# GonzaBerger/bmSparse-SPGEMM-SPMV

Hardware: AMD Instinct MI355X
Metric: bmSparse SpMV fp32 effective GB/s (CSR-convention bytes / time); SpGEMM GFLOP/s under `spgemm` (higher is better)
Workload: dtype f32; 1 GPU; bmSparse SpMV fp32, rmat(scale=20, edge_factor=2)+I, stand-in for webbase-1M; rows=1048576, nnz=3127380, blocks=2073692, x=ones, variant=default (value-stream sweep over the cached plan), hbm_resident_copies_rotated=9

## Files before the change

### bmsparse-spgemm-spmv_amd/csrc/spmv.hip

```cpp
#include "spmv_plan.h"
#include "prims.hip.h"
#include <cstdlib>
#include <cstdio>
#include <algorithm>
#include <vector>
#include <type_traits>

namespace bmsp {
namespace {

constexpr uint32_t kVsGroup = 96;
bool vstream_eligible(const bmsp_matrix_s *A)
{
    return !(A->spmv_full_tiles * 4 >= A->block_num) && !getenv("BMSP_SPMV_OLD") && A->num_block_cols() < (1ll << 28);
}

struct RowClass {
    const uint32_t *rowptr;
    const uint64_t *offsets;
    uint32_t nbr;
    uint32_t group;
    __device__ bool is_long(uint32_t r) const { return rowptr[r + 1] - rowptr[r] > kItemTiles; }
    __device__ bool starts(uint32_t r) const
    {
// ... 794 lines not shown
    constexpr int GROUPS = LANES_PER_ROW / 8;
    const uint32_t gid = blockIdx.x * (kThreads / LANES_PER_ROW) + threadIdx.x / LANES_PER_ROW;
    if (gid >= num_block_rows) return;
    const int sub = threadIdx.x % LANES_PER_ROW;
    const int g = sub >> 3, r = sub & 7;
    const uint32_t b0 = rowptr[gid], b1 = rowptr[gid + 1];
    A acc = 0;
    for (uint32_t b = b0 + g; b < b1; b += GROUPS) {
        uint64_t bmp = bmps[b];
        uint32_t byte = tile_byte(bmp, r);
        if (byte) {
            uint32_t before = r ? (uint32_t)__popcll(bmp >> (64 - 8 * r)) : 0u;
            acc = tile_row_dot<T, A>(byte, values + offsets[b] + before, x, key_col(keys[b]) * 8u, num_cols, acc);
        }
    }
    if (GROUPS > 1) {
#pragma unroll
        for (int d = 8; d < LANES_PER_ROW; d <<= 1) acc += __shfl_xor(acc, d, kWave);
    }
    uint32_t row = gid * 8u + (uint32_t)r;
    if (g == 0 && row >= row_lo && row < num_rows) y[row] = acc;
}

template <typename T, int U>
__global__ __launch_bounds__(kThreads) void spmv_rowgroup_kernel(const uint32_t *__restrict__ rowptr, const uint64_t *__restrict__ keys,
                                                                 const uint64_t *__restrict__ bmps, const uint64_t *__restrict__ offsets,
                                                                 const T *__restrict__ values, const T *__restrict__ x,
                                                                 typename Acc<T>::type *__restrict__ y, uint32_t num_rows, uint32_t num_cols,
                                                                 uint32_t nbr, uint32_t values_bytes, uint32_t passes, uint32_t row_lo)
{
    using A = typename Acc<T>::type;
    const int lane = lane_id(), j = lane & 15, g = lane >> 4;
    const uint32_t wv = blockIdx.x * 4 + wave_id();
    const rsrc_t rv = make_rsrc(values, values_bytes), rx = make_rsrc(x, num_cols * (uint32_t)sizeof(T));
    const uint32_t xlane = (uint32_t)((j & 1) * 4);
    const uint32_t bshift = (uint32_t)(60 - 4 * j) & 31u;
    const bool in_hi = j < 8;
    const uint32_t hi_mask = j >= 8 ? 0xffffffffu : (j == 0 ? 0u : 0xffffffffu << (32 - 4 * j));
    const uint32_t lo_mask = j > 8 ? 0xffffffffu << (64 - 4 * j) : 0u;
    const bool ragged_x = (num_cols & 3u) != 0u;
    for (uint32_t p = 0; p < passes; p++) {
        const uint32_t br = (wv * passes + p) * 4u + (uint32_t)g;
        if ((wv * passes + p) * 4u >= nbr) break;
        const bool valid = br < nbr;
        uint32_t t = valid ? rowptr[br] : 0u;
        const uint32_t t1 = valid ? rowptr[br + 1] : 0u;
        A acc = 0;
        uint32_t blo[U], bhi[U], col[U], off[U];
#pragma unroll
        for (int u = 0; u < U; u++) {
            const bool on = t + u < t1;
            const uint64_t bm = on ? bmps[t + u] : 0ull;
            blo[u] = (uint32_t)bm; bhi[u] = (uint32_t)(bm >> 32);
            col[u] = on ? (uint32_t)keys[t + u] : 0u;
            off[u] = on ? (uint32_t)offsets[t + u] : 0u;
        }
        while (__any(t < t1)) {
            A av[U][4], xv[U][4];
            uint32_t nib[U];
#pragma unroll
            for (int u = 0; u < U; u++) {
                nib[u] = ((in_hi ? bhi[u] : blo[u]) >> bshift) & 0xfu;
                const uint32_t rank = (uint32_t)__builtin_popcount(bhi[u] & hi_mask) + (uint32_t)__builtin_popcount(blo[u] & lo_mask);
                const uint32_t vaddr = (off[u] + rank) * (uint32_t)sizeof(T);
                if (sizeof(T) == 2) {
                    typedef uint32_t u32x3 __attribute__((ext_vector_type(3)));
                    typedef _Float16 h2 __attribute__((ext_vector_type(2)));
                    const u32x3 d = __builtin_amdgcn_raw_buffer_load_b96(rv, nib[u] ? (vaddr & ~3u) : kOob, 0, 0);
                    const uint32_t sh = (vaddr & 2u) * 8u;
                    const h2 p0 = __builtin_bit_cast(h2, __builtin_amdgcn_alignbit(d[1], d[0], sh)), p1 = __builtin_bit_cast(h2, __builtin_amdgcn_alignbit(d[2], d[1], sh));
                    av[u][0] = (A)p0[0]; av[u][1] = (A)p0[1]; av[u][2] = (A)p1[0]; av[u][3] = (A)p1[1];
                } else {
                    Buf4<T>::ld(rv, nib[u] ? vaddr : kOob, av[u]);
                }
                const uint32_t xc = col[u] * 8u + xlane;
                if (ragged_x && xc + 4u > num_cols) {
#pragma unroll
                    for (int q = 0; q < 4; q++) xv[u][q] = (A)Buf<T>::ld(rx, nib[u] && xc + q < num_cols ? (xc + q) * (uint32_t)sizeof(T) : kOob);
                } else {
                    Buf4<T>::ld(rx, nib[u] ? xc * (uint32_t)sizeof(T) : kOob, xv[u]);
                }
            }
            uint32_t nlo[U], nhi[U], ncol[U], noff[U];
#pragma unroll
            for (int u = 0; u < U; u++) {
                const bool on = t + U + u < t1;
                const uint64_t bm = on ? bmps[t + U + u] : 0ull;
                nlo[u] = (uint32_t)bm; nhi[u] = (uint32_t)(bm >> 32);
                ncol[u] = on ? (uint32_t)keys[t + U + u] : 0u;
                noff[u] = on ? (uint32_t)offsets[t + U + u] : 0u;
            }
#pragma unroll
            for (int u = 0; u < U; u++) {
                const uint32_t n = nib[u];
                A e0, e1, e2, e3;
                if (__all(n == 0xfu || n == 0u)) {
                    e0 = av[u][0]; e1 = av[u][1]; e2 = av[u][2]; e3 = av[u][3];
                    if (n == 0u) { e0 = e1 = e2 = e3 = A(0); }
                } else {
                    const bool b0 = n & 8u, b1 = n & 4u, b2 = n & 2u, b3 = n & 1u;
                    const uint32_t i2 = (uint32_t)b0 + (uint32_t)b1, i3 = i2 + (uint32_t)b2;
                    e0 = b0 ? av[u][0] : A(0);
                    e1 = b1 ? (b0 ? av[u][1] : av[u][0]) : A(0);
                    e2 = b2 ? (i2 == 0 ? av[u][0] : (i2 == 1 ? av[u][1] : av[u][2])) : A(0);
                    e3 = b3 ? (i3 == 0 ? av[u][0] : (i3 == 1 ? av[u][1] : (i3 == 2 ? av[u][2] : av[u][3]))) : A(0);
                }
                acc += e0 * xv[u][0] + e1 * xv[u][1] + e2 * xv[u][2] + e3 * xv[u][3];
            }
            t += U;
#pragma unroll
            for (int u = 0; u < U; u++) { blo[u] = nlo[u]; bhi[u] = nhi[u]; col[u] = ncol[u]; off[u] = noff[u]; }
        }
        if (sizeof(A) == 4) acc += __builtin_bit_cast(float, __builtin_amdgcn_update_dpp(0, __builtin_bit_cast(int, (float)acc), 0xB1, 0xf, 0xf, false));
        else acc += __shfl_xor(acc, 1, kWave);
        const uint32_t row = br * 8u + (uint32_t)(j >> 1);
        if (valid && !(j & 1) && row >= row_lo && row < num_rows) y[row] = acc;
    }
}

#ifndef BMSP_CH_V
#define BMSP_CH_V 512
#endif
constexpr uint32_t kChV = BMSP_CH_V;
constexpr int kChPer = (int)kChV / 64;
static_assert(kChPer % 4 == 0, "a lane loads its values four at a time");
constexpr uint32_t kChWin = 1024;
constexpr int64_t kChMinChunks = 128;
enum { kChHead = 1, kChTail = 2 };

struct ChunkRec {
    uint32_t fb;
    uint32_t own_b, own_e;
    uint32_t flags;
    uint32_t head_ca, head_cb;
    uint32_t tail_cb;
    uint32_t nwin;
};

__device__ __forceinline__ float chunk_sum8(const float (&s)[8], int lane)
{
    const bool h5 = lane & 32, h4 = lane & 16, h3 = lane & 8;
    float t[4], u[2];
#pragma unroll
    for (int i = 0; i < 4; i++) t[i] = (h5 ? s[i + 4] : s[i]) + __shfl_xor(h5 ? s[i] : s[i + 4], 32, kWave);
#pragma unroll
    for (int i = 0; i < 2; i++) u[i] = (h4 ? t[i + 2] : t[i]) + __shfl_xor(h4 ? t[i] : t[i + 2], 16, kWave);
    float v = (h3 ? u[1] : u[0]) + __shfl_xor(h3 ? u[0] : u[1], 8, kWave);
    v += __shfl_xor(v, 4, kWave);
    v += __shfl_xor(v, 2, kWave);
    v += __shfl_xor(v, 1, kWave);
    return v;
}

__device__ __forceinline__ void chunk_fold(const float *__restrict__ carry, float *__restrict__ y, uint32_t *__restrict__ counters, uint32_t ca,
                                           uint32_t cb, uint32_t br, uint32_t num_rows, int lane)
{
    const int r = lane & 7, g = lane >> 3;
    float sum = 0.f;
    for (uint32_t k = ca + (uint32_t)g; k <= cb; k += 8)
        sum += __hip_atomic_load(&carry[((size_t)k * 2 + (k == ca ? 1 : 0)) * 8 + r], __ATOMIC_RELAXED, __HIP_MEMORY_SCOPE_AGENT);
#pragma unroll
    for (int d = 8; d < 64; d <<= 1) sum += __shfl_xor(sum, d, kWave);
    const uint32_t row = br * 8u + (uint32_t)r;
    if (g == 0 && row < num_rows) y[row] = sum;
    if (lane == 0) __hip_atomic_store(&counters[ca], 0u, __ATOMIC_RELAXED, __HIP_MEMORY_SCOPE_AGENT);
}

__global__ __launch_bounds__(64, 8) void spmv_chunk_kernel(const ChunkRec *__restrict__ recs, const uint32_t *__restrict__ words,
                                                            const float *__restrict__ values, const float *__restrict__ x, float *__restrict__ y,
                                                            float *__restrict__ carry, uint32_t *__restrict__ counters, uint32_t nnz,
                                                            uint32_t num_rows, uint32_t num_cols, uint32_t colbits)
{
    typedef float f4 __attribute__((ext_vector_type(4)));
    typedef uint32_t u4 __attribute__((ext_vector_type(4)));
    __shared__ float win[kChWin];
    const int lane = lane_id();
    const uint32_t c = blockIdx.x;
    const ChunkRec rc = recs[c];
    const uint32_t first = c * kChV + (uint32_t)(kChPer * lane);
    const rsrc_t rw = make_rsrc(words, nnz * 4u), rv = make_rsrc(values, nnz * 4u), rx = make_rsrc(x, num_cols * 4u);
    uint32_t w[kChPer];
    float a[kChPer], xv[kChPer];
    if (c * kChV + kChV <= nnz) {
#pragma unroll
        for (int q = 0; q < kChPer; q += 4) {
            const u4 wq = __builtin_bit_cast(u4, __builtin_amdgcn_raw_buffer_load_b128(rw, (first + q) * 4u, 0, 0));
            const f4 aq = __builtin_bit_cast(f4, __builtin_amdgcn_raw_buffer_load_b128(rv, (first + q) * 4u, 0, 0));
#pragma unroll
            for (int i = 0; i < 4; i++) { w[q + i] = wq[i]; a[q + i] = aq[i]; }
        }
    } else {
#pragma unroll
        for (int j = 0; j < kChPer; j++) {
            const uint32_t off = first + j < nnz ? (first + j) * 4u : kOob;
            w[j] = __builtin_amdgcn_raw_buffer_load_b32(rw, off, 0, 0);
            a[j] = Buf<float>::ld(rv, off);
        }
    }
    const uint32_t cmask = (1u << colbits) - 1u;
#pragma unroll
    for (int j = 0; j < kChPer; j++) xv[j] = Buf<float>::ld(rx, first + j < nnz ? (w[j] & cmask) * 4u : kOob);

    float pr[kChPer];
    uint32_t rr[kChPer];
#pragma unroll
    for (int j = 0; j < kChPer; j++) {
        rr[j] = w[j] >> colbits;
        pr[j] = first + j < nnz ? a[j] * xv[j] : 0.f;
    }
    if (rc.nwin == 8) {
        float s[8] = {0.f, 0.f, 0.f, 0.f, 0.f, 0.f, 0.f, 0.f};
#pragma unroll
        for (int j = 0; j < kChPer; j++) {
#pragma unroll
            for (int k = 0; k < 8; k++) s[k] += rr[j] == (uint32_t)k ? pr[j] : 0.f;
        }
        const float v = chunk_sum8(s, lane);
        if ((lane & 7) == 0) win[((lane >> 5) & 1) * 4 + ((lane >> 4) & 1) * 2 + ((lane >> 3) & 1)] = v;
    } else {
        for (uint32_t e = (uint32_t)lane; e < rc.nwin; e += 64) win[e] = 0.f;
        __builtin_amdgcn_wave_barrier();
        float acc[kChPer];
        bool lead[kChPer];
#pragma unroll
        for (int j = 0; j < kChPer; j++) acc[j] = pr[j];
#pragma unroll
        for (int j = 0; j < kChPer; j++) {
            bool taken = false;
#pragma unroll
            for (int i = 0; i < j; i++) {
                const bool hit = !taken && rr[i] == rr[j];
                acc[i] += hit ? acc[j] : 0.f;
                taken |= hit;
            }
            lead[j] = !taken;
        }
#pragma unroll
        for (int j = 0; j < kChPer; j++)
            if (lead[j] && first + j < nnz) lds_add(win + rr[j], acc[j]);
    }
    __builtin_amdgcn_wave_barrier();
    const int32_t base = (int32_t)(rc.fb * 8u);
    const uint32_t row_end = min(rc.own_e * 8u, num_rows);
    for (uint32_t row = rc.own_b * 8u + (uint32_t)lane; row < row_end; row += 64) {
        const int32_t rel = (int32_t)row - base;
        y[row] = rel >= 0 && rel < (int32_t)rc.nwin ? win[rel] : 0.f;
    }
    if (!rc.flags) return;
    if ((rc.flags & kChHead) && lane < 8) __hip_atomic_store(&carry[((size_t)c * 2) * 8 + lane], win[lane], __ATOMIC_RELAXED, __HIP_MEMORY_SCOPE_AGENT);
    if ((rc.flags & kChTail) && lane < 8)
        __hip_atomic_store(&carry[((size_t)c * 2 + 1) * 8 + lane], win[rc.nwin - 8u + (uint32_t)lane], __ATOMIC_RELAXED, __HIP_MEMORY_SCOPE_AGENT);
    asm volatile("s_waitcnt vmcnt(0)" ::: "memory");
    uint32_t ticket = 0;
    if (lane == 0 && (rc.flags & kChHead)) ticket = __hip_atomic_fetch_add(&counters[rc.head_ca], 1u, __ATOMIC_RELAXED, __HIP_MEMORY_SCOPE_AGENT);
    if (lane == 1 && (rc.flags & kChTail)) ticket = __hip_atomic_fetch_add(&counters[c], 1u, __ATOMIC_RELAXED, __HIP_MEMORY_SCOPE_AGENT);
    const uint32_t th = (uint32_t)__builtin_amdgcn_readlane((int)ticket, 0), tt = (uint32_t)__builtin_amdgcn_readlane((int)ticket, 1);
    if ((rc.flags & kChHead) && th == rc.head_cb - rc.head_ca) chunk_fold(carry, y, counters, rc.head_ca, rc.head_cb, rc.fb, num_rows, lane);
    if ((rc.flags & kChTail) && tt == rc.tail_cb - c) chunk_fold(carry, y, counters, c, rc.tail_cb, rc.fb + rc.nwin / 8u - 1u, num_rows, lane);
}

__global__ void chunk_bounds_kernel(const uint64_t *__restrict__ keys, const uint64_t *__restrict__ bmps, const uint64_t *__restrict__ offsets,
                                    uint32_t nb, uint32_t nnz, uint32_t *__restrict__ fbr, uint32_t *__restrict__ lbr)
{
    const uint32_t b = blockIdx.x * blockDim.x + threadIdx.x;
    if (b >= nb) return;
    const uint32_t o = (uint32_t)offsets[b], n = (uint32_t)__popcll(bmps[b]);
    if (n == 0) return;
    const uint32_t br = key_row(keys[b]);
    for (uint32_t c = (o + kChV - 1) / kChV; c * kChV < o + n; c++) fbr[c] = br;
    for (uint32_t c = o / kChV; c <= (o + n - 1) / kChV; c++) {
        const uint32_t e = min((c + 1) * kChV, nnz) - 1u;
        if (e >= o && e < o + n) lbr[c] = br;
    }
}

__global__ void chunk_words_kernel(const uint64_t *__restrict__ keys, const uint64_t *__restrict__ bmps, const uint64_t *__restrict__ offsets,
                                   uint32_t nb, const uint32_t *__restrict__ fbr, uint32_t colbits, uint32_t *__restrict__ words)
{
    const uint32_t b = blockIdx.x * blockDim.x + threadIdx.x;
    if (b >= nb) return;
    uint64_t bm = bmps[b];
    const uint64_t k = keys[b];
    const uint32_t br = key_row(k), bc = key_col(k);
    uint32_t idx = (uint32_t)offsets[b];
    while (bm) {
        const uint32_t p = (uint32_t)__clzll((long long)bm);
        bm &= ~(0x8000000000000000ull >> p);
        const uint32_t rel = (br - fbr[idx / kChV]) * 8u + (p >> 3);
        words[idx] = (rel << colbits) | (bc * 8u + (p & 7u));
        idx++;
    }
}

void build_chunk_cache(bmsp_matrix_s *A, hipStream_t st)
{
    if (A->spmv_cw || A->spmv_cw_tried) return;
    A->spmv_cw_tried = 1;
    if (A->dtype != BMSP_F32 || A->view_values_end || A->view_block_begin || A->nnz == 0 || A->nnz >= (1ll << 30) || A->block_num == 0) return;
    if ((uintptr_t)A->values & 15u) return;
    const uint32_t nnz = (uint32_t)A->nnz, nb = (uint32_t)A->block_num;
    const uint32_t nch = (nnz + kChV - 1) / kChV;
    const int colbits = A->num_cols <= 1 ? 1 : 32 - __builtin_clz((uint32_t)A->num_cols - 1u);
    if (colbits > 28) return;
    std::vector<uint32_t> fb(nch), lb(nch);
    {
        DevBuf<uint32_t> d(2 * (size_t)nch);
        hipLaunchKernelGGL(chunk_bounds_kernel, dim3((nb + 255) / 256), dim3(256), 0, st, A->keys, A->bmps, A->offsets, nb, nnz, d.p, d.p + nch);
        BMSP_CHECK_LAUNCH();
        BMSP_HIP(hipStreamSynchronize(st));
        copy_d2h_staged(fb.data(), d.p, 4 * (size_t)nch);
        copy_d2h_staged(lb.data(), d.p + nch, 4 * (size_t)nch);
    }
    const uint64_t row_cap = std::min<uint64_t>(kChWin, 1ull << (32 - colbits));
    std::vector<ChunkRec> rec(nch);
    const uint32_t nbr = (uint32_t)A->num_block_rows();
    int64_t split = 0;
    for (uint32_t c = 0; c < nch; c++) {
        ChunkRec &r = rec[c];
        r.fb = fb[c];
        r.nwin = (lb[c] - fb[c] + 1u) * 8u;
        if (lb[c] < fb[c] || r.nwin > row_cap) return;
        const bool head = c > 0 && lb[c - 1] == fb[c], tail = c + 1 < nch && fb[c + 1] == lb[c];
        r.own_b = c == 0 ? 0u : fb[c] + (head ? 1u : 0u);
        r.own_e = c + 1 < nch ? fb[c + 1] : nbr;
        r.flags = (head ? kChHead : 0) | (tail && !(head && fb[c] == lb[c]) ? kChTail : 0);
        r.head_ca = r.head_cb = r.tail_cb = c;
    }
    for (uint32_t c = 0; c < nch; c++) {
        if (!(rec[c].flags & kChTail)) continue;
        split++;
        uint32_t e = c + 1;
        while (e + 1 < nch && fb[e + 1] == lb[c]) e++;
        rec[c].tail_cb = e;
        for (uint32_t k = c + 1; k <= e; k++) { rec[k].head_ca = c; rec[k].head_cb = e; }
    }
    const size_t off_rec = (size_t)nch * kChV * 4, off_cnt = off_rec + sizeof(ChunkRec) * (size_t)nch;
    const size_t off_carry = (off_cnt + 4 * (size_t)nch + 63) & ~size_t(63), total = off_carry + 64 * (size_t)nch;
    char *mem = (char *)pool_alloc(total);
    BMSP_HIP(hipMemsetAsync(mem, 0, total, st));
    BMSP_HIP(hipMemcpyAsync(mem + off_rec, rec.data(), sizeof(ChunkRec) * (size_t)nch, hipMemcpyHostToDevice, st));
    {
        DevBuf<uint32_t> d(nch);
        BMSP_HIP(hipMemcpyAsync(d.p, fb.data(), 4 * (size_t)nch, hipMemcpyHostToDevice, st));
        hipLaunchKernelGGL(chunk_words_kernel, dim3((nb + 255) / 256), dim3(256), 0, st, A->keys, A->bmps, A->offsets, nb, d.p, (uint32_t)colbits, (uint32_t *)mem);
        BMSP_CHECK_LAUNCH();
        BMSP_HIP(hipStreamSynchronize(st));
    }
    A->spmv_cw = (uint32_t *)mem;
    A->spmv_cw_chunks = nch;
    A->spmv_cw_split = split;
    A->spmv_cw_off_rec = off_rec; A->spmv_cw_off_cnt = off_cnt; A->spmv_cw_off_carry = off_carry;
    A->spmv_cw_colbits = colbits;
}

bool chunk_wanted(const bmsp_matrix_s *A, uint32_t row_lo, uint32_t row_hi)
{
    if (A->dtype != BMSP_F32 || row_lo != 0 || row_hi != (uint32_t)A->num_rows || A->view_values_end || A->view_block_begin) return false;
    if (getenv("BMSP_SPMV_NOCHUNK") || getenv("BMSP_SPMV_NO_POSCACHE") || getenv("BMSP_SPMV_RED")) return false;
    if (getenv("BMSP_SPMV_CHUNK")) return true;
    return A->nnz < 2 * A->block_num && (A->nnz + kChV - 1) / kChV >= kChMinChunks;
}

template <typename T>
void launch(bmsp_matrix_s *A, const void *v, void *u, int variant, hipStream_t st, uint32_t row_lo, uint32_t row_hi)
{
    using Ac = typename Acc<T>::type;
    uint32_t nbr = (uint32_t)A->num_block_rows();
    if (nbr == 0) return;
    if (variant == BMSP_SPMV_BATCHED) {
        hipLaunchKernelGGL((spmv_blockrow_kernel<T, 64>), dim3((nbr + 3) / 4), dim3(kThreads), 0, st, A->rowptr, A->keys, A->bmps,
                           A->offsets, (const T *)A->values, (const T *)v, (Ac *)u, row_hi,
                           (uint32_t)A->num_cols, nbr, row_lo);
    } else if (variant == 2) {
        hipLaunchKernelGGL((spmv_blockrow_kernel<T, 8>), dim3((nbr + 31) / 32), dim3(kThreads), 0, st, A->rowptr, A->keys, A->bmps,
                           A->offsets, (const T *)A->values, (const T *)v, (Ac *)u, row_hi,
                           (uint32_t)A->num_cols, nbr, row_lo);
    } else if ((size_t)A->values_extent() * sizeof(T) >= (1ull << 32) || (size_t)A->num_cols * sizeof(T) >= (1ull << 32)) {
        hipLaunchKernelGGL((spmv_blockrow_kernel<T, 64>), dim3((nbr + 3) / 4), dim3(kThreads), 0, st, A->rowptr, A->keys, A->bmps,
                           A->offsets, (const T *)A->values, (const T *)v, (Ac *)u, row_hi,
                           (uint32_t)A->num_cols, nbr, row_lo);
    } else {
        build_plan(A, st);
        const bool dense_tiles = A->block_num > 0 && A->nnz >= 16 * A->block_num;
        if ((variant == 3 || (variant == BMSP_SPMV_DEFAULT && dense_tiles && A->spmv_plan_long == 0 && !getenv("BMSP_SPMV_NO_ROWGROUP"))) && pool_owns(A->values)) {
            constexpr int U = 3;
            const uint32_t groups = (nbr + 3) / 4;
            const char *pe = getenv("BMSP_SPMV_PASSES");
            const uint32_t passes = pe ? (uint32_t)std::max(1, atoi(pe)) : (groups > 32768 ? 2u : 1u);
            const uint32_t waves = (groups + passes - 1) / passes;
            hipLaunchKernelGGL((spmv_rowgroup_kernel<T, U>), dim3((waves + 3) / 4), dim3(kThreads), 0, st, A->rowptr, A->keys, A->bmps, A->offsets,
                               (const T *)A->values, (const T *)v, (Ac *)u, row_hi, (uint32_t)A->num_cols, nbr,
                               (uint32_t)((size_t)A->values_extent() * sizeof(T)) + 16u, passes, row_lo);
// ... 145 lines not shown
```

Baseline: 2645 GB/s.

## Replace per-lane LDS atomic adds with DPP segmented reduction in chunk SpMV

In the multi-row chunk path, the per-lane O(kChPer^2) duplicate-combining loop followed by LDS atomic adds is replaced with a block-row (8-row) segmented reduction. Each lane builds 8-wide partial vectors per block row, runs a DPP-based segmented scan across the wave keyed on the last block row, and writes complete block rows to LDS with 16-byte vector stores instead of atomics. Out-of-range tail elements get a dummy row key so they do not break segments. This is meant to cut LDS atomic traffic and serialization, at the cost of more VALU and DPP work and an assumption that each lane's elements are sorted by row. A standalone experiment harness is also added that compares the two variants.

Result: faster. 2843 GB/s, median of 6 (+7.5%).

```diff
diff --git a/bmsparse-spgemm-spmv_amd/csrc/spmv.hip b/bmsparse-spgemm-spmv_amd/csrc/spmv.hip
--- a/bmsparse-spgemm-spmv_amd/csrc/spmv.hip
+++ b/bmsparse-spgemm-spmv_amd/csrc/spmv.hip
@@ -970,6 +970,65 @@
     return v;
 }
 
+__device__ __forceinline__ void chunk_put8(float *p, const float (&v)[8])
+{
+    typedef float f4 __attribute__((ext_vector_type(4)));
+    *(f4 *)p = f4{v[0], v[1], v[2], v[3]};
+    *(f4 *)(p + 4) = f4{v[4], v[5], v[6], v[7]};
+}
+
+template <int CTRL, int ROWS>
+__device__ __forceinline__ bool chunk_scan_step(float (&t)[8], uint32_t key)
+{
+    const bool m = dpp_u32<CTRL, ROWS>(~0u, key) == key;
+    if (!__builtin_amdgcn_ballot_w64(m)) return false;
+#pragma unroll
+    for (int k = 0; k < 8; k++) {
+        const float n = t[k] + dpp_val<CTRL, ROWS>(0.f, t[k]);
+        t[k] = m ? n : t[k];
+    }
+    return true;
+}
+
+__device__ __forceinline__ void chunk_seg_reduce(float *win, const uint32_t (&rk)[kChPer], const float (&pr)[kChPer])
+{
+    const uint32_t bf = rk[0] >> 3, bl = rk[kChPer - 1] >> 3;
+    float h[8], t[8];
+#pragma unroll
+    for (int k = 0; k < 8; k++) h[k] = t[k] = 0.f;
+#pragma unroll
+    for (int j = 0; j < kChPer; j++) {
+        if (j > 0 && (rk[j] >> 3) != (rk[j - 1] >> 3)) {
+            const uint32_t bp = rk[j - 1] >> 3;
+            if (bp == bf) {
+#pragma unroll
+                for (int k = 0; k < 8; k++) h[k] = t[k];
+            } else {
+                chunk_put8(win + 8u * bp, t);
+            }
+#pragma unroll
+            for (int k = 0; k < 8; k++) t[k] = 0.f;
+        }
+        const uint32_t r = rk[j] & 7u;
+#pragma unroll
+        for (int k = 0; k < 8; k++) t[k] += r == (uint32_t)k ? pr[j] : 0.f;
+    }
+    if (chunk_scan_step<0x111, 0xf>(t, bl) && chunk_scan_step<0x112, 0xf>(t, bl) && chunk_scan_step<0x114, 0xf>(t, bl)) chunk_scan_step<0x118, 0xf>(t, bl);
+    chunk_scan_step<0x142, 0xa>(t, bl);
+    chunk_scan_step<0x143, 0xc>(t, bl);
+    const uint32_t bl_left = dpp_u32<0x138>(~0u, bl), bf_right = dpp_u32<0x130>(~0u, bf);
+    float tl[8];
+#pragma unroll
+    for (int k = 0; k < 8; k++) tl[k] = dpp_val<0x138>(0.f, t[k]);
+    if (bf != bl) {
+        const bool cont = bl_left == bf;
+#pragma unroll
+        for (int k = 0; k < 8; k++) h[k] = cont ? h[k] + tl[k] : h[k];
+        chunk_put8(win + 8u * bf, h);
+    }
+    if (bf_right != bl) chunk_put8(win + 8u * bl, t);
+}
+
 __device__ __forceinline__ void chunk_fold(const float *__restrict__ carry, float *__restrict__ y, uint32_t *__restrict__ counters, uint32_t ca,
                                            uint32_t cb, uint32_t br, uint32_t num_rows, int lane)
 {
@@ -991,7 +1050,7 @@
 {
     typedef float f4 __attribute__((ext_vector_type(4)));
     typedef uint32_t u4 __attribute__((ext_vector_type(4)));
-    __shared__ float win[kChWin];
+    __shared__ __attribute__((aligned(16))) float win[kChWin];
     const int lane = lane_id();
     const uint32_t c = blockIdx.x;
     const ChunkRec rc = recs[c];
@@ -1023,7 +1082,7 @@
     uint32_t rr[kChPer];
 #pragma unroll
     for (int j = 0; j < kChPer; j++) {
-        rr[j] = w[j] >> colbits;
+        rr[j] = first + j < nnz ? w[j] >> colbits : rc.nwin - 8u;
         pr[j] = first + j < nnz ? a[j] * xv[j] : 0.f;
     }
     if (rc.nwin == 8) {
@@ -1038,24 +1097,7 @@
     } else {
         for (uint32_t e = (uint32_t)lane; e < rc.nwin; e += 64) win[e] = 0.f;
         __builtin_amdgcn_wave_barrier();
-        float acc[kChPer];
-        bool lead[kChPer];
-#pragma unroll
-        for (int j = 0; j < kChPer; j++) acc[j] = pr[j];
-#pragma unroll
-        for (int j = 0; j < kChPer; j++) {
-            bool taken = false;
-#pragma unroll
-            for (int i = 0; i < j; i++) {
-                const bool hit = !taken && rr[i] == rr[j];
-                acc[i] += hit ? acc[j] : 0.f;
-                taken |= hit;
-            }
-            lead[j] = !taken;
-        }
-#pragma unroll
-        for (int j = 0; j < kChPer; j++)
-            if (lead[j] && first + j < nnz) lds_add(win + rr[j], acc[j]);
+        chunk_seg_reduce(win, rr, pr);
     }
     __builtin_amdgcn_wave_barrier();
     const int32_t base = (int32_t)(rc.fb * 8u);
diff --git a/experiments/spmv_chunk_segscan.hip b/experiments/spmv_chunk_segscan.hip
--- /dev/null
+++ b/experiments/spmv_chunk_segscan.hip
@@ -0,0 +1,405 @@
+#include <hip/hip_runtime.h>
+#include <algorithm>
+#include <cmath>
+#include <cstdint>
+#include <cstdio>
+#include <vector>
+
+constexpr uint32_t kV = 512, kPer = kV / 64, kWin = 1024, kOob = 0xffffffffu;
+enum { kHead = 1, kTail = 2 };
+struct Rec { uint32_t fb, own_b, own_e, flags, head_ca, head_cb, tail_cb, nwin; };
+typedef __amdgpu_buffer_rsrc_t rsrc_t;
+typedef float f4 __attribute__((ext_vector_type(4)));
+typedef uint32_t u4 __attribute__((ext_vector_type(4)));
+
+__device__ __forceinline__ rsrc_t rsrc(const void *p, uint32_t bytes) { return __builtin_amdgcn_make_buffer_rsrc(const_cast<void *>(p), 0, bytes, 0x00020000); }
+__device__ __forceinline__ float ldf(rsrc_t r, uint32_t off) { return __builtin_bit_cast(float, __builtin_amdgcn_raw_buffer_load_b32(r, off, 0, 0)); }
+
+__device__ __forceinline__ float sum8(const float (&s)[8], int lane)
+{
+    const bool h5 = lane & 32, h4 = lane & 16, h3 = lane & 8;
+    float t[4], u[2];
+#pragma unroll
+    for (int i = 0; i < 4; i++) t[i] = (h5 ? s[i + 4] : s[i]) + __shfl_xor(h5 ? s[i] : s[i + 4], 32, 64);
+#pragma unroll
+    for (int i = 0; i < 2; i++) u[i] = (h4 ? t[i + 2] : t[i]) + __shfl_xor(h4 ? t[i] : t[i + 2], 16, 64);
+    float v = (h3 ? u[1] : u[0]) + __shfl_xor(h3 ? u[0] : u[1], 8, 64);
+    v += __shfl_xor(v, 4, 64);
+    v += __shfl_xor(v, 2, 64);
+    v += __shfl_xor(v, 1, 64);
+    return v;
+}
+
+__device__ __forceinline__ void fold(const float *carry, float *y, uint32_t *counters, uint32_t ca, uint32_t cb, uint32_t br, uint32_t num_rows, int lane)
+{
+    const int r = lane & 7, g = lane >> 3;
+    float sum = 0.f;
+    for (uint32_t k = ca + (uint32_t)g; k <= cb; k += 8)
+        sum += __hip_atomic_load(&carry[((size_t)k * 2 + (k == ca ? 1 : 0)) * 8 + r], __ATOMIC_RELAXED, __HIP_MEMORY_SCOPE_AGENT);
+#pragma unroll
+    for (int d = 8; d < 64; d <<= 1) sum += __shfl_xor(sum, d, 64);
+    const uint32_t row = br * 8u + (uint32_t)r;
+    if (g == 0 && row < num_rows) y[row] = sum;
+    if (lane == 0) __hip_atomic_store(&counters[ca], 0u, __ATOMIC_RELAXED, __HIP_MEMORY_SCOPE_AGENT);
+}
+
+__device__ __forceinline__ void load_chunk(uint32_t c, int lane, const uint32_t *words, const float *values, const float *x, uint32_t nnz,
+                                           uint32_t num_cols, uint32_t (&w)[kPer], float (&a)[kPer], float (&xv)[kPer])
+{
+    const uint32_t first = c * kV + kPer * (uint32_t)lane;
+    const rsrc_t rw = rsrc(words, nnz * 4u), rv = rsrc(values, nnz * 4u), rx = rsrc(x, num_cols * 4u);
+    if (c * kV + kV <= nnz) {
+#pragma unroll
+        for (uint32_t q = 0; q < kPer; q += 4) {
+            const u4 wq = __builtin_bit_cast(u4, __builtin_amdgcn_raw_buffer_load_b128(rw, (first + q) * 4u, 0, 0));
+            const f4 aq = __builtin_bit_cast(f4, __builtin_amdgcn_raw_buffer_load_b128(rv, (first + q) * 4u, 0, 0));
+#pragma unroll
+            for (int i = 0; i < 4; i++) { w[q + i] = wq[i]; a[q + i] = aq[i]; }
+        }
+    } else {
+#pragma unroll
+        for (uint32_t j = 0; j < kPer; j++) {
+            const uint32_t off = first + j < nnz ? (first + j) * 4u : kOob;
+            w[j] = __builtin_amdgcn_raw_buffer_load_b32(rw, off, 0, 0);
+            a[j] = ldf(rv, off);
+        }
+    }
+#pragma unroll
+    for (uint32_t j = 0; j < kPer; j++) xv[j] = ldf(rx, first + j < nnz ? (w[j] & 0xfffffu) * 4u : kOob);
+}
+
+template <int R, bool CMB = false>
+__global__ __launch_bounds__(64, 8) void r5_kernel(const Rec *recs, const uint32_t *words, const float *values, const float *x, float *y, float *out,
+                                                   float *carry, uint32_t *counters, uint32_t nnz, uint32_t num_rows, uint32_t num_cols)
+{
+    __shared__ float win[kWin];
+    const int lane = threadIdx.x & 63;
+    const uint32_t c = blockIdx.x;
+    const Rec rc = recs[c];
+    const uint32_t first = c * kV + kPer * (uint32_t)lane;
+    uint32_t w[kPer];
+    float a[kPer], xv[kPer];
+    load_chunk(c, lane, words, values, x, nnz, num_cols, w, a, xv);
+    if (rc.nwin == 8) {
+        float s[8] = {0.f, 0.f, 0.f, 0.f, 0.f, 0.f, 0.f, 0.f};
+#pragma unroll
+        for (uint32_t j = 0; j < kPer; j++) {
+            const uint32_t rr = w[j] >> 20;
+            const float p = first + j < nnz ? a[j] * xv[j] : 0.f;
+#pragma unroll
+            for (int k = 0; k < 8; k++) s[k] += rr == (uint32_t)k ? p : 0.f;
+        }
+        const float v = sum8(s, lane);
+        if ((lane & 7) == 0) win[((lane >> 5) & 1) * 4 + ((lane >> 4) & 1) * 2 + ((lane >> 3) & 1)] = v;
+    } else {
+        for (uint32_t e = (uint32_t)lane; e < rc.nwin; e += 64) win[e] = 0.f;
+        __builtin_amdgcn_wave_barrier();
+        if constexpr (CMB) {
+            float acc[kPer];
+            bool lead[kPer];
+#pragma unroll
+            for (uint32_t j = 0; j < kPer; j++) acc[j] = first + j < nnz ? a[j] * xv[j] : 0.f;
+#pragma unroll
+            for (uint32_t j = 0; j < kPer; j++) {
+                bool taken = false;
+#pragma unroll
+                for (uint32_t i = 0; i < j; i++) {
+                    const bool hit = !taken && (w[i] >> 20) == (w[j] >> 20);
+                    acc[i] += hit ? acc[j] : 0.f;
+                    taken |= hit;
+                }
+                lead[j] = !taken;
+            }
+#pragma unroll
+            for (uint32_t j = 0; j < kPer; j++)
+                if (lead[j] && first + j < nnz) __hip_atomic_fetch_add(win + (w[j] >> 20), acc[j], __ATOMIC_RELAXED, __HIP_MEMORY_SCOPE_WAVEFRONT);
+        }
+        float run = 0.f;
+#pragma unroll
+        for (uint32_t j = 0; j < kPer && !CMB; j++) {
+            const uint32_t rr = w[j] >> 20;
+            const bool on = first + j < nnz;
+            const bool flush = j == kPer - 1 || first + j + 1 >= nnz || (w[j + (j < kPer - 1 ? 1 : 0)] >> 20) != rr;
+            run += on ? a[j] * xv[j] : 0.f;
+            if (flush) {
+                if (on) __hip_atomic_fetch_add(win + rr, run, __ATOMIC_RELAXED, __HIP_MEMORY_SCOPE_WAVEFRONT);
+                run = 0.f;
+            }
+        }
+    }
+    __builtin_amdgcn_wave_barrier();
+    if constexpr (R == 2) {
+        out[c * 64 + lane] = win[lane & 7];
+        return;
+    }
+    const int32_t base = (int32_t)(rc.fb * 8u);
+    const uint32_t row_end = min(rc.own_e * 8u, num_rows);
+    for (uint32_t row = rc.own_b * 8u + (uint32_t)lane; row < row_end; row += 64) {
+        const int32_t rel = (int32_t)row - base;
+        y[row] = rel >= 0 && rel < (int32_t)rc.nwin ? win[rel] : 0.f;
+    }
+    if (R == 3 || !rc.flags) return;
+    if ((rc.flags & kHead) && lane < 8) __hip_atomic_store(&carry[((size_t)c * 2) * 8 + lane], win[lane], __ATOMIC_RELAXED, __HIP_MEMORY_SCOPE_AGENT);
+    if ((rc.flags & kTail) && lane < 8)
+        __hip_atomic_store(&carry[((size_t)c * 2 + 1) * 8 + lane], win[rc.nwin - 8u + (uint32_t)lane], __ATOMIC_RELAXED, __HIP_MEMORY_SCOPE_AGENT);
+    asm volatile("s_waitcnt vmcnt(0)" ::: "memory");
+    if constexpr (R == 4) return;
+    uint32_t ticket = 0;
+    if (lane == 0 && (rc.flags & kHead)) ticket = __hip_atomic_fetch_add(&counters[rc.head_ca], 1u, __ATOMIC_RELAXED, __HIP_MEMORY_SCOPE_AGENT);
+    if (lane == 1 && (rc.flags & kTail)) ticket = __hip_atomic_fetch_add(&counters[c], 1u, __ATOMIC_RELAXED, __HIP_MEMORY_SCOPE_AGENT);
+    const uint32_t th = (uint32_t)__builtin_amdgcn_readlane((int)ticket, 0), tt = (uint32_t)__builtin_amdgcn_readlane((int)ticket, 1);
+    if constexpr (R == 5) {
+        if (th == kOob && tt == kOob) out[c * 64 + lane] = 0.f;
+        return;
+    }
+    if ((rc.flags & kHead) && th == rc.head_cb - rc.head_ca) fold(carry, y, counters, rc.head_ca, rc.head_cb, rc.fb, num_rows, lane);
+    if ((rc.flags & kTail) && tt == rc.tail_cb - c) fold(carry, y, counters, c, rc.tail_cb, rc.fb + rc.nwin / 8u - 1u, num_rows, lane);
+}
+
+template <int CTRL, int ROWS = 0xf>
+__device__ __forceinline__ float dppf(float old, float v)
+{
+    return __builtin_bit_cast(float, __builtin_amdgcn_update_dpp(__builtin_bit_cast(int, old), __builtin_bit_cast(int, v), CTRL, ROWS, 0xf, false));
+}
+template <int CTRL, int ROWS = 0xf>
+__device__ __forceinline__ uint32_t dppu(uint32_t old, uint32_t v) { return (uint32_t)__builtin_amdgcn_update_dpp((int)old, (int)v, CTRL, ROWS, 0xf, false); }
+
+__device__ __forceinline__ void put8(float *p, const float (&v)[8])
+{
+    *(f4 *)p = f4{v[0], v[1], v[2], v[3]};
+    *(f4 *)(p + 4) = f4{v[4], v[5], v[6], v[7]};
+}
+
+template <int CTRL, int ROWS>
+__device__ __forceinline__ bool seg_step(float (&t)[8], uint32_t key)
+{
+    const bool m = dppu<CTRL, ROWS>(~0u, key) == key;
+    if (!__builtin_amdgcn_ballot_w64(m)) return false;
+#pragma unroll
+    for (int k = 0; k < 8; k++) {
+        const float n = t[k] + dppf<CTRL, ROWS>(0.f, t[k]);
+        t[k] = m ? n : t[k];
+    }
+    return true;
+}
+
+__device__ __forceinline__ void seg_reduce(float *win, const uint32_t (&rk)[kPer], const float (&pr)[kPer])
+{
+    const uint32_t bf = rk[0] >> 3, bl = rk[kPer - 1] >> 3;
+    float h[8], t[8];
+#pragma unroll
+    for (int k = 0; k < 8; k++) h[k] = t[k] = 0.f;
+#pragma unroll
+    for (uint32_t j = 0; j < kPer; j++) {
+        if (j > 0 && (rk[j] >> 3) != (rk[j - 1] >> 3)) {
+            const uint32_t bp = rk[j - 1] >> 3;
+            if (bp == bf) {
+#pragma unroll
+                for (int k = 0; k < 8; k++) h[k] = t[k];
+            } else {
+                put8(win + 8u * bp, t);
+            }
+#pragma unroll
+            for (int k = 0; k < 8; k++) t[k] = 0.f;
+        }
+        const uint32_t r = rk[j] & 7u;
+#pragma unroll
+        for (int k = 0; k < 8; k++) t[k] += r == (uint32_t)k ? pr[j] : 0.f;
+    }
+    if (seg_step<0x111, 0xf>(t, bl) && seg_step<0x112, 0xf>(t, bl) && seg_step<0x114, 0xf>(t, bl)) seg_step<0x118, 0xf>(t, bl);
+    seg_step<0x142, 0xa>(t, bl);
+    seg_step<0x143, 0xc>(t, bl);
+    const uint32_t bl_left = dppu<0x138>(~0u, bl), bf_right = dppu<0x130>(~0u, bf);
+    float tl[8];
+#pragma unroll
+    for (int k = 0; k < 8; k++) tl[k] = dppf<0x138>(0.f, t[k]);
+    if (bf != bl) {
+        const bool cont = bl_left == bf;
+#pragma unroll
+        for (int k = 0; k < 8; k++) h[k] = cont ? h[k] + tl[k] : h[k];
+        put8(win + 8u * bf, h);
+    }
+    if (bf_right != bl) put8(win + 8u * bl, t);
+}
+
+__global__ __launch_bounds__(64, 8) void r7_kernel(const Rec *recs, const uint32_t *words, const float *values, const float *x, float *y,
+                                                   float *carry, uint32_t *counters, uint32_t nnz, uint32_t num_rows, uint32_t num_cols)
+{
+    __shared__ __attribute__((aligned(16))) float win[kWin];
+    const int lane = threadIdx.x & 63;
+    const uint32_t c = blockIdx.x;
+    const Rec rc = recs[c];
+    const uint32_t first = c * kV + kPer * (uint32_t)lane;
+    uint32_t w[kPer];
+    float a[kPer], xv[kPer];
+    load_chunk(c, lane, words, values, x, nnz, num_cols, w, a, xv);
+    float pr[kPer];
+    uint32_t rr[kPer];
+#pragma unroll
+    for (uint32_t j = 0; j < kPer; j++) {
+        rr[j] = first + j < nnz ? w[j] >> 20 : rc.nwin - 8u;
+        pr[j] = first + j < nnz ? a[j] * xv[j] : 0.f;
+    }
+    if (rc.nwin == 8) {
+        float s[8] = {0.f, 0.f, 0.f, 0.f, 0.f, 0.f, 0.f, 0.f};
+#pragma unroll
+        for (uint32_t j = 0; j < kPer; j++)
+#pragma unroll
+            for (int k = 0; k < 8; k++) s[k] += rr[j] == (uint32_t)k ? pr[j] : 0.f;
+        const float v = sum8(s, lane);
+        if ((lane & 7) == 0) win[((lane >> 5) & 1) * 4 + ((lane >> 4) & 1) * 2 + ((lane >> 3) & 1)] = v;
+    } else {
+        for (uint32_t e = (uint32_t)lane; e < rc.nwin; e += 64) win[e] = 0.f;
+        __builtin_amdgcn_wave_barrier();
+        seg_reduce(win, rr, pr);
+    }
+    __builtin_amdgcn_wave_barrier();
+    const int32_t base = (int32_t)(rc.fb * 8u);
+    const uint32_t row_end = min(rc.own_e * 8u, num_rows);
+    for (uint32_t row = rc.own_b * 8u + (uint32_t)lane; row < row_end; row += 64) {
+        const int32_t rel = (int32_t)row - base;
+        y[row] = rel >= 0 && rel < (int32_t)rc.nwin ? win[rel] : 0.f;
+    }
+    if (!rc.flags) return;
+    if ((rc.flags & kHead) && lane < 8) __hip_atomic_store(&carry[((size_t)c * 2) * 8 + lane], win[lane], __ATOMIC_RELAXED, __HIP_MEMORY_SCOPE_AGENT);
+    if ((rc.flags & kTail) && lane < 8)
+        __hip_atomic_store(&carry[((size_t)c * 2 + 1) * 8 + lane], win[rc.nwin - 8u + (uint32_t)lane], __ATOMIC_RELAXED, __HIP_MEMORY_SCOPE_AGENT);
+    asm volatile("s_waitcnt vmcnt(0)" ::: "memory");
+    uint32_t ticket = 0;
+    if (lane == 0 && (rc.flags & kHead)) ticket = __hip_atomic_fetch_add(&counters[rc.head_ca], 1u, __ATOMIC_RELAXED, __HIP_MEMORY_SCOPE_AGENT);
+    if (lane == 1 && (rc.flags & kTail)) ticket = __hip_atomic_fetch_add(&counters[c], 1u, __ATOMIC_RELAXED, __HIP_MEMORY_SCOPE_AGENT);
+    const uint32_t th = (uint32_t)__builtin_amdgcn_readlane((int)ticket, 0), tt = (uint32_t)__builtin_amdgcn_readlane((int)ticket, 1);
+    if ((rc.flags & kHead) && th == rc.head_cb - rc.head_ca) fold(carry, y, counters, rc.head_ca, rc.head_cb, rc.fb, num_rows, lane);
+    if ((rc.flags & kTail) && tt == rc.tail_cb - c) fold(carry, y, counters, c, rc.tail_cb, rc.fb + rc.nwin / 8u - 1u, num_rows, lane);
+}
+
+#define CK(x)                                                                                 \
+    do {                                                                                      \
+        hipError_t e_ = (x);                                                                  \
+        if (e_ != hipSuccess) { printf("HIP error %s at line %d\n", hipGetErrorString(e_), __LINE__); return 1; } \
+    } while (0)
+
+int main()
+{
+    const uint32_t scale = 20, n = 1u << scale, m = 2u << scale, copies = 9;
+    uint64_t z = 12345;
+    auto next = [&z]() { z = z * 6364136223846793005ull + 1442695040888963407ull; return (double)(z >> 11) * (1.0 / 9007199254740992.0); };
+    std::vector<uint64_t> cells;
+    for (uint32_t e = 0; e < m + n; e++) {
+        uint32_t r = 0, c = 0;
+        if (e < m) {
+            for (uint32_t l = 0; l < scale; l++) {
+                const double u = next();
+                r = (r << 1) | (u >= 0.76 ? 1u : 0u);
+                c = (c << 1) | (((u >= 0.57 && u < 0.76) || u >= 0.95) ? 1u : 0u);
+            }
+        } else {
+            r = c = e - m;
+        }
+        cells.push_back(((uint64_t)(r >> 3) << 43) | ((uint64_t)(c >> 3) << 26) | ((uint64_t)(((r & 7u) << 3) | (c & 7u)) << 20) | c);
+    }
+    std::sort(cells.begin(), cells.end());
+    cells.erase(std::unique(cells.begin(), cells.end()), cells.end());
+    const uint32_t nnz = (uint32_t)cells.size(), nch = (nnz + kV - 1) / kV, nbr = n / 8;
+    auto brow = [&](uint32_t i) { return (uint32_t)(cells[i] >> 43); };
+    std::vector<uint32_t> fb(nch), lb(nch);
+    for (uint32_t c = 0; c < nch; c++) { fb[c] = brow(c * kV); lb[c] = brow(std::min((c + 1) * kV, nnz) - 1); }
+    std::vector<Rec> rec(nch);
+    uint32_t hub = 0, folded = 0;
+    for (uint32_t c = 0; c < nch; c++) {
+        Rec &r = rec[c];
+        r.fb = fb[c];
+        r.nwin = (lb[c] - fb[c] + 1u) * 8u;
+        if (r.nwin > kWin) { printf("chunk %u spans %u rows: beyond the window\n", c, r.nwin); return 1; }
+        const bool head = c > 0 && lb[c - 1] == fb[c], tail = c + 1 < nch && fb[c + 1] == lb[c];
+        r.own_b = c == 0 ? 0u : fb[c] + (head ? 1u : 0u);
+        r.own_e = c + 1 < nch ? fb[c + 1] : nbr;
+        r.flags = (head ? kHead : 0) | (tail && !(head && fb[c] == lb[c]) ? kTail : 0);
+        r.head_ca = r.head_cb = r.tail_cb = c;
+        hub += r.nwin == 8;
+        folded += r.flags != 0;
+    }
+    for (uint32_t c = 0; c < nch; c++) {
+        if (!(rec[c].flags & kTail)) continue;
+        uint32_t e = c + 1;
+        while (e + 1 < nch && fb[e + 1] == lb[c]) e++;
+        rec[c].tail_cb = e;
+        for (uint32_t k = c + 1; k <= e; k++) { rec[k].head_ca = c; rec[k].head_cb = e; }
+    }
+    std::vector<uint32_t> hw((size_t)nch * kV, 0);
+    std::vector<float> hv((size_t)nch * kV, 0.f), hx(n);
+    for (uint32_t i = 0; i < nnz; i++) {
+        const uint32_t rel = (brow(i) - fb[i / kV]) * 8u + (uint32_t)((cells[i] >> 23) & 7u);
+        hw[i] = (rel << 20) | (uint32_t)(cells[i] & 0xfffffu);
+        hv[i] = (float)(0.25 + 0.5 * next());
+    }
+    for (uint32_t i = 0; i < n; i++) hx[i] = (float)(0.5 + next());
+    std::vector<double> yref(n, 0.0);
+    for (uint32_t i = 0; i < nnz; i++) yref[brow(i) * 8u + ((cells[i] >> 23) & 7u)] += (double)hv[i] * hx[cells[i] & 0xfffffu];
+    printf("nnz %u, chunks %u, hub chunks %u, chunks that fold %u\n", nnz, nch, hub, folded);
+
+    uint32_t *dw[copies], *dcnt;
+    float *dv[copies], *dx, *dy, *dout, *dcarry;
+    Rec *drec;
+    for (uint32_t c = 0; c < copies; c++) {
+        CK(hipMalloc((void **)&dw[c], 4ull * hw.size())); CK(hipMemcpy(dw[c], hw.data(), 4ull * hw.size(), hipMemcpyHostToDevice));
+        CK(hipMalloc((void **)&dv[c], 4ull * hv.size())); CK(hipMemcpy(dv[c], hv.data(), 4ull * hv.size(), hipMemcpyHostToDevice));
+    }
+    CK(hipMalloc((void **)&dx, 4ull * n)); CK(hipMemcpy(dx, hx.data(), 4ull * n, hipMemcpyHostToDevice));
+    CK(hipMalloc((void **)&dy, 4ull * n));
+    CK(hipMalloc((void **)&dout, 4ull * nch * 64));
+    CK(hipMalloc((void **)&dcarry, 64ull * nch));
+    CK(hipMalloc((void **)&dcnt, 4ull * nch));
+    CK(hipMalloc((void **)&drec, sizeof(Rec) * nch)); CK(hipMemcpy(drec, rec.data(), sizeof(Rec) * nch, hipMemcpyHostToDevice));
+    hipEvent_t e0, e1;
+    CK(hipEventCreate(&e0)); CK(hipEventCreate(&e1));
+    const int warm = 20, reps = 200;
+    auto timed = [&](const char *name, auto launch) -> int {
+        CK(hipMemset(dcnt, 0, 4ull * nch));
+        for (int it = 0; it < warm; it++) launch(it % copies);
+        CK(hipEventRecord(e0, 0));
+        for (int it = 0; it < reps; it++) launch(it % copies);
+        CK(hipEventRecord(e1, 0));
+        CK(hipEventSynchronize(e1));
+        CK(hipGetLastError());
+        float ms = 0;
+        CK(hipEventElapsedTime(&ms, e0, e1));
+        printf("%-44s %7.2f us per launch\n", name, ms * 1e3 / reps);
+        return 0;
+    };
+#define L(...) [&](int k) { hipLaunchKernelGGL(__VA_ARGS__); }
+    const char *names[2] = {"j  round-6 kernel (window adds)", "k  j + segmented reduction"};
+    auto variant = [&](int v, const char *name) -> int {
+        switch (v) {
+        case 0: return timed(name, L((r5_kernel<6, true>), dim3(nch), dim3(64), 0, 0, drec, dw[k], dv[k], dx, dy, dout, dcarry, dcnt, nnz, n, n));
+        default: return timed(name, L(r7_kernel, dim3(nch), dim3(64), 0, 0, drec, dw[k], dv[k], dx, dy, dcarry, dcnt, nnz, n, n));
+        }
+    };
+    std::vector<std::vector<float>> ys;
+    for (int v = 0; v < 2; v++) {
+        CK(hipMemset(dy, 0xff, 4ull * n));
+        if (variant(v, names[v])) return 1;
+        std::vector<float> h(n);
+        CK(hipMemcpy(h.data(), dy, 4ull * n, hipMemcpyDeviceToHost));
+        double worst = 0;
+        uint32_t bad = 0;
+        for (uint32_t i = 0; i < n; i++) {
+            if (!std::isfinite(h[i])) bad++;
+            worst = std::max(worst, std::fabs(h[i] - yref[i]) / std::max(1e-30, std::fabs(yref[i])));
+        }
+        uint32_t differ = 0;
+        double wf = 0;
+        for (uint32_t i = 0; v > 0 && i < n; i++) {
+            if (h[i] != ys[0][i]) differ++;
+            wf = std::max(wf, (double)std::fabs(h[i] - ys[0][i]) / std::max(1e-30, std::fabs((double)ys[0][i])));
+        }
+        printf("   non-finite rows %u; largest relative error against the host sum %.3g; against j: %u rows differ, largest relative difference %.3g\n",
+               bad, worst, differ, wf);
+        if (bad || worst > 1e-5) { printf("   WRONG\n"); return 2; }
+        ys.push_back(h);
+    }
+    for (int rep = 0; rep < 4; rep++)
+        for (int v = 0; v < 2; v++)
+            if (variant(v, names[v])) return 1;
+    return 0;
+}
```
